# bytedance/particle-sfm

Hardware: AMD Instinct MI355X
Metric: trajectory-points/s (higher is better)
Workload: dtype f32 sampling + f64 positions; 1 GPU; configs[1]: synthetic 100x(1920x1080) flow pairs, sample_ratio=2, flow_check + chaining + occlusion + id assignment, 1 sequence per GPU; frames=101, height=1080, width=1920, trajectories=2073277, parallelism=sequence-per-gpu x1, world_size=1

## Files before the change

### include/psfm.h

```cpp
#ifndef PSFM_H_
#define PSFM_H_

#include <stddef.h>
#include <stdint.h>

#ifdef __cplusplus
extern "C" {
#endif

#define PSFM_VERSION 141

typedef enum psfm_status {
    PSFM_OK = 0,
    PSFM_ERR_ARG = 1,
    PSFM_ERR_HIP = 2,
    PSFM_ERR_CAPACITY = 3,
    PSFM_ERR_SOLVER = 4
} psfm_status;

typedef struct psfm_ctx psfm_ctx;

enum {
    PSFM_TERM_FUNCTION_TOL = 0,
    PSFM_TERM_PARAMETER_TOL = 1,
// ... 45 lines not shown
                                int w, const float* thres, int pair0, int n_pairs, uint8_t* const* kill_out, void* stream);

psfm_status psfm_ctx_set_solver(psfm_ctx* ctx, int mode, int k);
psfm_status psfm_solver_counters(psfm_ctx* ctx, int64_t* fused, int64_t* fused_redone, int64_t* chain, int32_t* k_now);

psfm_status psfm_ctx_set_resident_budget(psfm_ctx* ctx, int blocks);
psfm_status psfm_resident_capacity(psfm_ctx* ctx, int32_t* blocks);

psfm_status psfm_solver_launches(psfm_ctx* ctx, int64_t* resident, int64_t* giveups, int64_t* iterations);

psfm_status psfm_flow_check(psfm_ctx* ctx, const float* flows_f, const float* flows_b, int n_pairs, int h,
                            int w, float thres, uint8_t* occ_out, float* err_out, void* stream);

psfm_status psfm_load_flo_stack(psfm_ctx* ctx, const char* const* paths_host, int n, int h, int w, float* dst, int n_threads, void* stream);

psfm_status psfm_grid_sample(psfm_ctx* ctx, const float* map_hwc, int c, int h, int w, const double* xy,
                             int64_t n, float* out, void* stream);

psfm_status psfm_optimize_location(psfm_ctx* ctx, const double* uv12, const double* ref1, const double* ref2,
                                   const double* scale, const float* flow12, int64_t n, int w, int h,
                                   double* out, psfm_solve_stats* stats_host, void* stream);

psfm_status psfm_path_consistency_eval(psfm_ctx* ctx, const double* uv12, const double* ref1, const double* ref2,
                                       const double* scale, const float* flow12, int64_t n, int w, int h,
                                       double* residuals, double* jacobians, void* stream);

psfm_status psfm_sort_records(psfm_ctx* ctx, uint32_t* keys, int32_t* values, int64_t n, int end_bit, void* stream);

psfm_status psfm_sort_records64(psfm_ctx* ctx, uint64_t* keys, int32_t* values, int64_t n, int end_bit, void* stream);

psfm_status psfm_ctx_get_finalize_forms(psfm_ctx* ctx, int* sort_form, int* offsets_form);

psfm_status psfm_ctx_get_finalize_placed(psfm_ctx* ctx, int* placed);

psfm_status psfm_track(psfm_ctx* ctx, const float* flows, const uint8_t* occ, const float* flows_f2,
                       const uint8_t* occ_s2, int n_flows, int h, int w, int sample_ratio,
                       psfm_track_info* info_host, void* stream);

psfm_status psfm_connect(psfm_ctx* ctx, const float* flows_f, const float* flows_b, const float* flows_f2,
                         const float* flows_b2, int n_flows, int h, int w, float thres, int sample_ratio,
                         uint8_t* occ, uint8_t* occ_s2, psfm_track_info* info_host, void* stream);

psfm_status psfm_track_queries(psfm_ctx* ctx, const float* flows_f, const uint8_t* occ_f, const float* flows_b, const uint8_t* occ_b,
                               int n_flows, int h, int w, const double* q_xy, const int32_t* q_t, int64_t n_q,
                               psfm_track_info* info_host, void* stream);

psfm_status psfm_track_queries_optimize(psfm_ctx* ctx, const float* flows_f, const uint8_t* occ_f, const float* flows_f2,
                                        const uint8_t* occ_f2, const float* flows_b, const uint8_t* occ_b, const float* flows_b2,
                                        const uint8_t* occ_b2, int n_flows, int h, int w, const double* q_xy, const int32_t* q_t,
                                        int64_t n_q, psfm_track_info* info_host, void* stream);

psfm_status psfm_track_queries_batch(psfm_ctx* const* ctxs, int n_seq, const float* const* flows_f, const uint8_t* const* occ_f,
                                     const float* const* flows_b, const uint8_t* const* occ_b, const int* n_flows, const int* h,
                                     const int* w, const double* const* q_xy, const int32_t* const* q_t, const int64_t* n_q,
                                     psfm_track_info* infos_host, void* stream);
psfm_status psfm_query_batch_census(psfm_ctx* ctx, int32_t* launches, int32_t* host_syncs);

psfm_status psfm_track_queries_optimize_batch(psfm_ctx* const* ctxs, int n_seq, const float* const* flows_f, const uint8_t* const* occ_f,
                                              const float* const* flows_f2, const uint8_t* const* occ_f2, const float* const* flows_b,
                                              const uint8_t* const* occ_b, const float* const* flows_b2, const uint8_t* const* occ_b2,
                                              const int* n_flows, const int* h, const int* w, const double* const* q_xy,
                                              const int32_t* const* q_t, const int64_t* n_q, psfm_track_info* infos_host, void* stream);
psfm_status psfm_query_pc_batch_census(psfm_ctx* ctx, int32_t* launches_fixed, int32_t* launches_iter, int32_t* host_syncs);

psfm_status psfm_connect_batch(psfm_ctx* const* ctxs, int n_seq, const float* const* flows_f, const float* const* flows_b,
                               const float* const* flows_f2, const float* const* flows_b2, const int* n_flows, int h, int w,
// ... 151 lines not shown
```

### particle-sfm_amd/csrc/psfm_api.hip

```cpp
#include <stdarg.h>
#include <stdio.h>
#include <string.h>
#include <mutex>
#include <shared_mutex>
#include <atomic>
#include <chrono>
#include <stdlib.h>

#include "psfm_internal.h"
#include "psfm_solve_policy.h"

static thread_local char g_err[512] = "";
static std::shared_mutex g_dev_gate[16];
std::shared_mutex& psfm_device_gate(int device) { return g_dev_gate[device & 15]; }
static std::atomic<int> g_dev_waiters[16];
int psfm_gate_waiters(int device) { return g_dev_waiters[device & 15].load(std::memory_order_relaxed); }
void psfm_gate_waiters_add(int device, int d) { g_dev_waiters[device & 15].fetch_add(d, std::memory_order_relaxed); }
static int psfm_wants_persist(psfm_ctx* c, bool optimize, int h, int w, int ratio, bool fused)
{
    if (c->chain_mode == 1 || ratio < 1 || !psfm_frame_ok(h, w)) return 0;
    if (c->mb_enable && !optimize) return 0;
    if (optimize) return c->resident_budget > 0 ? 0 : 1;
    const int64_t G = (int64_t)((w + ratio - 1) / ratio) * ((h + ratio - 1) / ratio);
    const int64_t P = (int64_t)h * w;
// ... 351 lines not shown
        return PSFM_ERR_ARG;
    }
    if (n == 0) return PSFM_OK;
    hipStream_t s = (hipStream_t)stream;
    psfm_status st;
    if ((st = c->sort_keys.ensure(sizeof(unsigned long long) * (size_t)n * 2)) != PSFM_OK) return st;
    if ((st = c->sort_lanes.ensure(sizeof(int) * (size_t)n * 2)) != PSFM_OK) return st;
    const int64_t half = psfm_sort_pairs64_passes((unsigned)end_bit) % 2 == 0 ? 0 : n;
    unsigned long long* k0 = c->sort_keys.as<unsigned long long>();
    int* v0 = c->sort_lanes.as<int>();
    PSFM_HIP(hipMemcpyAsync(k0 + half, keys, sizeof(unsigned long long) * (size_t)n, hipMemcpyDeviceToDevice, s));
    PSFM_HIP(hipMemcpyAsync(v0 + half, values, sizeof(int) * (size_t)n, hipMemcpyDeviceToDevice, s));
    if ((st = psfm_sort_pairs64(c, k0, v0, k0 + n, v0 + n, n, (unsigned)end_bit, s)) != PSFM_OK) return st;
    PSFM_HIP(hipMemcpyAsync(keys, k0, sizeof(unsigned long long) * (size_t)n, hipMemcpyDeviceToDevice, s));
    PSFM_HIP(hipMemcpyAsync(values, v0, sizeof(int) * (size_t)n, hipMemcpyDeviceToDevice, s));
    return PSFM_OK;
}

extern "C" psfm_status psfm_ctx_get_finalize_forms(psfm_ctx* c, int* sort_form, int* offsets_form)
{
    PSFM_CHECK_CTX(c);
    if (sort_form) *sort_form = c->fin_sort_form;
    if (offsets_form) *offsets_form = c->fin_offsets_form;
    return PSFM_OK;
}

extern "C" psfm_status psfm_ctx_get_finalize_placed(psfm_ctx* c, int* placed)
{
    PSFM_CHECK_CTX(c);
    if (placed) *placed = c->fin_placed;
    return PSFM_OK;
}

psfm_status psfm_track_dims(psfm_ctx* c, int n_flows, int h, int w, int ratio, int64_t g_own, PsfmTrackDims& d)
{
    d.H = h; d.W = w; d.ratio = ratio; d.n_flows = n_flows;
    d.GW = (w + ratio - 1) / ratio; d.GH = (h + ratio - 1) / ratio;
    d.G = (int64_t)d.GW * d.GH;
    const int64_t Gown = g_own < 0 ? d.G : (g_own > 0 ? g_own : 1);
    d.cap = (int64_t)(c->lane_factor * (double)Gown);
    d.cap = ((d.cap + 255) / 256) * 256;
    const int64_t n_blocks = d.cap / 256;
    {
        const int64_t gb = (Gown + 255) / 256;
        d.nsh = (int)(gb < PSFM_NSHARD ? (gb > 0 ? gb : 1) : PSFM_NSHARD);
    }
    d.free_cap = (int)(((n_blocks + d.nsh - 1) / d.nsh) * 256) + 1024;
    const double tf = c->traj_factor > (double)n_flows / 8.0 ? c->traj_factor : (double)n_flows / 8.0;
    d.shard_cap = (int)(((int64_t)(tf * (double)Gown) + d.cap) / d.nsh) + 1024;
    d.traj_cap = (int64_t)d.shard_cap * PSFM_NSHARD;
    if (d.cap > 0x7fffffff / 2 || d.traj_cap > 0x7fffffff / 2) { psfm_set_error("psfm_track: grid too large"); return PSFM_ERR_ARG; }
    d.shift_b = 1; while ((1ll << d.shift_b) < d.G) ++d.shift_b;
    int tbits = 1; while ((1ll << tbits) < (long long)n_flows + 2) ++tbits;
    d.shift_d = d.shift_b + tbits;
    if (d.shift_d + tbits > 63) { psfm_set_error("psfm_track: key does not fit 64 bits"); return PSFM_ERR_ARG; }
    d.cw = (float)((double)(w - 1) / 2.0); d.ch = (float)((double)(h - 1) / 2.0);
    return PSFM_OK;
}

psfm_status psfm_track_alloc(psfm_ctx* c, const PsfmTrackDims& d)
{
    psfm_status st;
    const int n_flows = d.n_flows;
    if ((st = c->log.ensure(sizeof(double2) * (size_t)(n_flows + 1) * d.cap)) != PSFM_OK) return st;
    if ((st = c->birth_frame.ensure(sizeof(int) * d.cap)) != PSFM_OK) return st;
    if ((st = c->birth_idx.ensure(sizeof(int) * d.cap)) != PSFM_OK) return st;
// ... 429 lines not shown
```

### particle-sfm_amd/csrc/psfm_finalize.hip

```cpp
#include <cstring>
#include <stdio.h>
#include <rocprim/device/device_radix_sort.hpp>
#include <rocprim/device/device_scan.hpp>

#include "psfm_device.h"
#include "psfm_finalize_plan.h"
#include "psfm_internal.h"
#include "psfm_place.h"

#define PSFM_BLOCK 256

__device__ __forceinline__ void psfm_collect_alive_body(
    const int* __restrict__ birth_frame, const int* __restrict__ birth_idx, PsfmCounters* __restrict__ ctr,
    PsfmShard* __restrict__ shards, unsigned long long* __restrict__ fin_keys, int* __restrict__ fin_lanes, int cap,
    int shard_cap, int last_time, int shift_b, int shift_d)
{
    __shared__ int s_cnt[PSFM_BLOCK / PSFM_WAVE];
    __shared__ int s_base;
    const int n_lanes = min(ctr->n_lanes, cap);
    if ((int)(blockIdx.x * PSFM_BLOCK) >= n_lanes) return;
    const int i = blockIdx.x * PSFM_BLOCK + threadIdx.x;
    int bf = -1;
    if (i < n_lanes) bf = birth_frame[i];
    const bool pending = bf <= -2;
    const bool alive = (bf >= 0) | pending;
    const int my_last = pending ? last_time - 1 : last_time;
    if (pending) bf = -2 - bf;
    const unsigned long long am = __ballot(alive);
    const int lane = psfm_lane_id(), wave = threadIdx.x / PSFM_WAVE;
    if (lane == 0) s_cnt[wave] = __popcll(am);
    __syncthreads();
    const int shard = blockIdx.x % PSFM_NSHARD;
    if (threadIdx.x == 0) {
        int tot = 0;
        for (int w = 0; w < PSFM_BLOCK / PSFM_WAVE; ++w) tot += s_cnt[w];
        s_base = tot > 0 ? atomicAdd(&shards[shard].fin_cnt, tot) : 0;
    }
    __syncthreads();
    if (alive) {
// ... 280 lines not shown
        r[u] = (t >= 1 && t < lj) ? dlog[(int64_t)(bj + t - 1) * cap + col] : make_float2(0.f, 0.f);
    }
    if (tid < TILE_J) s_off[tid] = id0 + tid < n ? psfm_track_offset(pl, off, id0 + tid, hb, hl) : 0;
    for (int k0 = 0; k0 < maxlen; k0 += TILE_K) {
#pragma unroll
        for (int u = 0; u < NLD; ++u) dtile[j][q + u * (PSFM_BLOCK / TILE_J)] = r[u];
        __syncthreads();
        if (k0 + TILE_K < maxlen) {
#pragma unroll
            for (int u = 0; u < NLD; ++u) {
                const int t = k0 + TILE_K + q + u * (PSFM_BLOCK / TILE_J);
                r[u] = (t < lj) ? dlog[(int64_t)(bj + t - 1) * cap + col] : make_float2(0.f, 0.f);
            }
        }
        if (tid < TILE_J) {
            double2 pos = s_pos[tid];
            const int l = s_len[tid];
            float2 f[TILE_K];
#pragma unroll
            for (int k = 0; k < TILE_K; ++k) f[k] = dtile[tid][k];
#pragma unroll
            for (int k = 0; k < TILE_K; ++k) {
                const int t = k0 + k;
                if (t >= 1 && t < l) { pos.x = pos.x + (double)f[k].x; pos.y = pos.y + (double)f[k].y; }
                tile[tid][k] = pos;
            }
            s_pos[tid] = pos;
        }
        __syncthreads();
        const int kk = tid & (TILE_K - 1);
        for (int jj = tid / TILE_K; jj < TILE_J; jj += PSFM_BLOCK / TILE_K) {
            const int t = k0 + kk;
            if (t < s_len[jj]) out[s_off[jj] + t] = tile[jj][kk];
        }
        __syncthreads();
    }
}

static PsfmFinForm psfm_form_of(const PsfmTrackDims& d, int64_t n, int n_seq = 0)
{
    static const int sort_on = getenv("PSFM_FIN_SORT") ? atoi(getenv("PSFM_FIN_SORT")) : 1;
    static const int plan_on = getenv("PSFM_FIN_PLAN") ? atoi(getenv("PSFM_FIN_PLAN")) : 1;
    return psfm_fin_form(d.shift_b, d.shift_d, d.n_flows, n_seq > 0 ? n_seq : 1, n, sort_on, plan_on, n_seq > 0 ? 0 : 1);
}

struct PsfmFinDst { unsigned long long* keys; int* lanes; };
static PsfmFinDst psfm_compact_dst(psfm_ctx* c, const PsfmFinForm& f, int64_t n)
{
    const int64_t half = f.first_half ? 0 : n;
    return {f.fmt.use32 ? (unsigned long long*)(c->sort_keys.as<unsigned>() + half) : c->sort_keys.as<unsigned long long>() + half,
            c->sort_lanes.as<int>() + half};
}

template <class K>
static psfm_status psfm_rocprim_sort(psfm_ctx* c, int64_t n, unsigned end_bit, size_t scan_bytes, hipStream_t s)
{
    K* k_out = c->sort_keys.as<K>(), *k_in = k_out + n;
    int* l_out = c->sort_lanes.as<int>(), *l_in = l_out + n;
    size_t tmp_bytes = 0;
    psfm_status st;
    PSFM_HIP(rocprim::radix_sort_pairs(nullptr, tmp_bytes, k_in, k_out, l_in, l_out, (size_t)n, 0u, end_bit, s));
    if ((st = c->sort_tmp.ensure(tmp_bytes > scan_bytes ? tmp_bytes : scan_bytes)) != PSFM_OK) return st;
    PSFM_HIP(rocprim::radix_sort_pairs(c->sort_tmp.p, tmp_bytes, k_in, k_out, l_in, l_out, (size_t)n, 0u, end_bit, s));
    return PSFM_OK;
}

// ... 43 lines not shown
    const long long ng = f.ng;
    const PsfmKeyFmt fmt = f.fmt;
    PsfmPlan pl;
    pl.gstart = nullptr; pl.goff = nullptr; pl.keys = (const void*)c->sort_keys.p; pl.use32 = fmt.use32; pl.shift_b = d.shift_b; pl.shift_d = d.shift_d;
    pl.birth_w = c->res_birth.as<int>(); pl.len_w = c->res_len.as<int>(); pl.off_w = c->res_off.as<int64_t>();
    if (f.offsets_form == 1) {
        if ((st = c->scan_tmp.ensure((sizeof(int64_t) + sizeof(int)) * (size_t)ng)) != PSFM_OK) return st;
        int64_t* goff = c->scan_tmp.as<int64_t>();
        int* gstart = (int*)(goff + ng);
        const void* had = c->fin_marks.p;
        if ((st = c->fin_marks.ensure(sizeof(int) * (size_t)PSFM_PLAN_MAX_GROUPS)) != PSFM_OK) return st;
        if (!c->fin_marks_clean || had != c->fin_marks.p)
            PSFM_HIP(hipMemsetAsync(c->fin_marks.p, 0xff, sizeof(int) * (size_t)PSFM_PLAN_MAX_GROUPS, s));
        c->fin_marks_clean = false;
        hipLaunchKernelGGL(psfm_group_bounds_kernel, dim3((unsigned)((n + PSFM_BLOCK - 1) / PSFM_BLOCK)), dim3(PSFM_BLOCK), 0, s,
                           (const void*)c->sort_keys.p, n, fmt.use32, d.shift_b, d.shift_d, c->fin_marks.as<int>());
        hipLaunchKernelGGL(psfm_group_plan_kernel, dim3(1), dim3(PSFM_PLAN_BLOCK), 0, s, c->fin_marks.as<int>(), gstart, goff, (int)ng, n,
                           c->res_off.as<int64_t>() + n);
        PSFM_HIP(hipGetLastError());
        c->fin_marks_clean = true;
        c->fin_offsets_form = 1;
        pl.gstart = gstart; pl.goff = goff;
    } else {
        c->fin_offsets_form = 3;
        if ((st = c->scan_tmp.ensure(sizeof(int64_t) * (n + 1))) != PSFM_OK) return st;
        hipLaunchKernelGGL(psfm_decode_kernel, dim3((unsigned)((n + 1 + PSFM_BLOCK - 1) / PSFM_BLOCK)), dim3(PSFM_BLOCK), 0, s,
                           (const void*)c->sort_keys.p, n, fmt, c->res_birth.as<int>(), c->res_len.as<int>(), c->scan_tmp.as<int64_t>());
        PSFM_HIP(hipGetLastError());
        PSFM_HIP(rocprim::exclusive_scan(c->sort_tmp.p, scan_bytes, c->scan_tmp.as<int64_t>(), c->res_off.as<int64_t>(),
                                         (int64_t)0, (size_t)(n + 1), rocprim::plus<int64_t>(), s));
    }
    c->res_n_points = npts;
    if ((st = c->res_xy.ensure(sizeof(double2) * (size_t)(npts > 0 ? npts : 1))) != PSFM_OK) return st;
    if (delta_log)
        hipLaunchKernelGGL(psfm_gather_delta_kernel, dim3((unsigned)((n + TILE_J - 1) / TILE_J)), dim3(PSFM_BLOCK), 0, s,
                           c->log.as<float2>(), d.cap, c->sort_lanes.as<int>(), c->res_birth.as<int>(),
                           c->res_len.as<int>(), c->res_off.as<int64_t>(), n, (const void*)c->sort_keys.p, fmt.use32,
                           d.shift_b, d.GW, d.ratio, c->res_xy.as<double2>(), pl);
    else
        hipLaunchKernelGGL(psfm_gather_kernel, dim3((unsigned)((n + TILE_J - 1) / TILE_J)), dim3(PSFM_BLOCK), 0, s,
                           c->log.as<double2>(), d.cap, c->sort_lanes.as<int>(), c->res_birth.as<int>(),
                           c->res_len.as<int>(), c->res_off.as<int64_t>(), n, c->res_xy.as<double2>(), pl);
    PSFM_HIP(hipGetLastError());
    return PSFM_OK;
}

psfm_status psfm_finalize(psfm_ctx* c, const PsfmTrackDims& d, hipStream_t s)
{
    PsfmCounters* ctr = c->counters.as<PsfmCounters>();
    PsfmShard* shards = c->shards.as<PsfmShard>();
    hipLaunchKernelGGL(psfm_collect_alive_kernel, dim3((unsigned)((d.cap + PSFM_BLOCK - 1) / PSFM_BLOCK)), dim3(PSFM_BLOCK),
                       0, s, c->birth_frame.as<int>(), c->birth_idx.as<int>(), ctr, shards,
                       c->fin_keys.as<unsigned long long>(), c->fin_lanes.as<int>(), (int)d.cap, d.shard_cap,
                       d.n_flows, d.shift_b, d.shift_d);
    PSFM_HIP(hipGetLastError());
    PsfmCounters* hc = (PsfmCounters*)c->host_pinned;
    PsfmShard* hs = psfm_host_shards(c);
    PSFM_HIP(hipMemcpyAsync(hc, ctr, sizeof(PsfmCounters), hipMemcpyDeviceToHost, s));
    PSFM_HIP(hipMemcpyAsync(hs, shards, sizeof(PsfmShard) * PSFM_NSHARD, hipMemcpyDeviceToHost, s));
    PSFM_HIP(hipStreamSynchronize(s));
    PsfmShardOffsets so;
    int fin_cnt[PSFM_NSHARD];
    int64_t n = 0, npts = 0;
    for (int k = 0; k < PSFM_NSHARD; ++k) { npts += hs[k].points; fin_cnt[k] = hs[k].fin_cnt; }
    const bool over = psfm_shard_offsets(fin_cnt, d.shard_cap, &so, &n) || hc->overflow != 0;
    if (over || hc->n_lanes > d.cap) {
        psfm_set_error("capacity exceeded: lanes used %d of %lld, trajectory records %lld of %lld (%d shards); "
                       "raise psfm_ctx_set_capacity", hc->n_lanes, (long long)d.cap, (long long)n,
                       (long long)d.traj_cap, PSFM_NSHARD);
        return PSFM_ERR_CAPACITY;
    }
    c->res_n_traj = n;
// ... 270 lines not shown
```

### particle-sfm_amd/csrc/psfm_internal.h

```cpp
#pragma once
#include <hip/hip_runtime.h>
#include <stdint.h>
#include <string.h>
#include <shared_mutex>
#include <string>
#include <vector>

#include "../../include/psfm.h"

#define PSFM_MAX_PEERS 8

void psfm_set_error(const char* fmt, ...);

#define PSFM_HIP(expr)                                                                          \
    do {                                                                                        \
        hipError_t e_ = (expr);                                                                 \
        if (e_ != hipSuccess) {                                                                 \
            psfm_set_error("%s failed: %s (%s:%d)", #expr, hipGetErrorString(e_), __FILE__, __LINE__); \
            return PSFM_ERR_HIP;                                                                \
        }                                                                                       \
    } while (0)

static inline bool psfm_frame_ok(int h, int w) { return h >= 2 && w >= 2 && (int64_t)h * (int64_t)w * 8 < ((int64_t)1 << 32); }

// ... 81 lines not shown

struct PsfmTrackDims;

struct psfm_ctx {
    int device = 0;
    double lane_factor = 2.0, traj_factor = 8.0;
    PsfmBuf log;
    PsfmBuf birth_frame;
    PsfmBuf birth_idx;
    PsfmBuf free_stack;
    PsfmBuf fin_keys;
    PsfmBuf fin_lanes;
    PsfmBuf occupied;
    PsfmBuf counters;
    PsfmBuf shards;
    PsfmBuf survivors;
    PsfmBuf handoff;
    PsfmBuf seg_info;
    PsfmBuf seg_table;
    PsfmBuf persist_bar;
    PsfmBuf place_tab;
    int persist_max_blocks = -1;
    int chain_mode = 0;
    bool mb_enable = false;
    float mb_thres = 0.02f;
    PsfmBuf kill;
    void* host_seg = nullptr;
    size_t host_seg_bytes = 0;
    PsfmBuf sort_keys, sort_lanes, sort_tmp, scan_tmp;
    PsfmBuf fin_marks;
    bool fin_marks_clean = false;
    int fin_sort_form = 0, fin_offsets_form = 0;
    int fin_placed = 0;
    PsfmBuf res_birth, res_len, res_off, res_xy;
    int64_t res_n_traj = 0, res_n_points = 0;
    int res_n_flows = 0;
    bool res_is_query = false;
    PsfmBuf qr_ws;
    PsfmBuf qb_tab, qb_ws;
    void* qb_host = nullptr;
    int32_t qb_launches = 0, qb_syncs = 0;
    PsfmBuf qpb_tab, qpb_ws, qpb_owner;
    void* qpb_host = nullptr;
    int32_t qpb_fixed = 0, qpb_iter = 0, qpb_syncs = 0;
    PsfmBuf sol_x, sol_state, sol_partials, sol_ctrl, sol_misc, sol_stats, sol_fused, sol_bar;
    PsfmBuf sol_list;
    int pc_persist_blocks[4] = {-1, -1, -1, -1};
    bool pc_persist_ok = false;
    int resident_budget = 0;
    unsigned pc_epoch = 0;
    PsfmBuf peer_area;
    unsigned peer_epoch = 0;
    int peer_world = 0, peer_rank = 0;
    int peer_L[PSFM_MAX_PEERS] = {0};
    void* peer_lead[PSFM_MAX_PEERS] = {nullptr};
    void* peer_opened[PSFM_MAX_PEERS] = {nullptr};
    int pc_giveups = 0;
    int solve_K = 4;
    int solve_mode = 0;
    int solver_mode = 0, solver_K = 0;
    int64_t n_fused_ok = 0, n_fused_redone = 0, n_chain = 0;
    int64_t n_resident = 0, n_iter_launches = 0;
    PsfmTrackDims* shard_dims = nullptr;
    bool shard_optimize = false;
    int solve_unroll = 6;
    PsfmBuf occ_own, occ2_own;
// ... 286 lines not shown
```

### particle-sfm_amd/point_trajectory/_hip.py

```python
import ctypes
import os

_PKG = os.path.dirname(os.path.dirname(os.path.abspath(__file__)))
LIB_PATH = os.environ.get("PSFM_HIP_LIB", os.path.join(_PKG, "lib", "libpsfm_hip.so"))

PSFM_OK, PSFM_ERR_ARG, PSFM_ERR_HIP, PSFM_ERR_CAPACITY, PSFM_ERR_SOLVER = 0, 1, 2, 3, 4
PROF_KINDS = {"flow_check": 0, "chain_step": 1, "respawn": 2, "solver": 3, "finalize": 4}

EXPORTS = [
    "psfm_last_error", "psfm_version", "psfm_device_count", "psfm_ctx_create", "psfm_ctx_destroy",
    "psfm_ctx_set_capacity", "psfm_flow_check", "psfm_grid_sample", "psfm_optimize_location", "psfm_track",
    "psfm_connect",
    "psfm_result_device", "psfm_result_copy", "psfm_result_solve_stats", "psfm_ctx_set_profiling",
    "psfm_profile_get", "psfm_ctx_set_chain_mode", "psfm_window_sample", "psfm_result_filter", "psfm_result_filtered_copy",
    "psfm_ctx_set_solver", "psfm_solver_counters", "psfm_traj_to_matches", "psfm_matches_copy",
    "psfm_shard_begin", "psfm_shard_step", "psfm_shard_solve_export", "psfm_shard_solve_control", "psfm_shard_solve_restore",
    "psfm_shard_solve_writeback", "psfm_shard_solve_record", "psfm_shard_finish", "psfm_result_keys",
    "psfm_shard_solve_control_async", "psfm_shard_window_state", "psfm_shard_peek_stall", "psfm_shard_frame",
    "psfm_shard_solve_control_chain_async", "psfm_shard_solve_poll", "psfm_shard_solve_local", "psfm_shard_solve_redo_local", "psfm_connect_batch", "psfm_solver_launches", "psfm_ctx_set_resident_budget", "psfm_resident_capacity", "psfm_load_flo_stack",
    "psfm_path_consistency_eval", "psfm_sort_records", "psfm_sort_records64", "psfm_ctx_get_finalize_forms", "psfm_ctx_get_finalize_placed",
    "psfm_shard_peer_area", "psfm_shard_peer_epoch", "psfm_shard_peer_open", "psfm_shard_peer_connect", "psfm_shard_solve_blocks", "psfm_shard_solve_peer",
    "psfm_labels_begin", "psfm_labels_merge_window", "psfm_labels_finish", "psfm_labels_device", "psfm_labels_copy", "psfm_labels_to_matches",
    "psfm_traj_augment", "psfm_traj_encode_weight_count", "psfm_traj_encode",
    "psfm_traj_decode_weight_count", "psfm_traj_decode_workspace_bytes", "psfm_traj_decode",
    "psfm_traj_decode_batch_workspace_bytes", "psfm_traj_decode_batch",
    "psfm_window_sample_batch", "psfm_traj_augment_batch", "psfm_traj_encode_batch",
    "psfm_traj_eval_counts", "psfm_traj_vote_labels",
    "psfm_labels_set", "psfm_matches_to_database", "psfm_database_copy", "psfm_database_chunk_rows",
    "psfm_database_compact_again",
    "psfm_sparse_depth", "psfm_sparse_depth_sort_ids", "psfm_ctx_set_sparse_depth", "psfm_ctx_get_sparse_depth_budget",
    "psfm_sparse_depth_last_ms", "psfm_colmap_points3d_count", "psfm_colmap_points3d_scan",
    "psfm_ctx_set_motion_boundary", "psfm_motion_boundary", "psfm_kill_map", "psfm_kill_map_batch",
    "psfm_depth_display", "psfm_ctx_set_depth_display", "psfm_depth_display_last_ms", "psfm_depth_display_chunk",
    "psfm_track_queries", "psfm_track_queries_optimize",
    "psfm_result_filter_batch", "psfm_traj_to_matches_batch", "psfm_labels_to_matches_batch", "psfm_matches_batch_census", "psfm_labels_sizes",
    "psfm_track_queries_batch", "psfm_query_batch_census",
    "psfm_track_queries_optimize_batch", "psfm_query_pc_batch_census",
    "psfm_ctx_set_batch_redo", "psfm_connect_batch_census", "psfm_ctx_set_frame_size",
]


class SolveStats(ctypes.Structure):
    _fields_ = [("iterations", ctypes.c_int32), ("successful_steps", ctypes.c_int32),
                ("termination", ctypes.c_int32), ("dogleg_nonGN", ctypes.c_int32),
                ("initial_cost", ctypes.c_double), ("final_cost", ctypes.c_double)]

    def as_dict(self):
        return {k: getattr(self, k) for k, _ in self._fields_}


class TrackInfo(ctypes.Structure):
    _fields_ = [("n_traj", ctypes.c_int64), ("n_points", ctypes.c_int64), ("n_lanes_peak", ctypes.c_int64),
                ("lane_capacity", ctypes.c_int64), ("solver_iterations", ctypes.c_int64),
                ("n_solves", ctypes.c_int32), ("chain_mode", ctypes.c_int32)]

    def as_dict(self):
        return {k: getattr(self, k) for k, _ in self._fields_}


class PsfmError(RuntimeError):
    def __init__(self, status, msg):
        super().__init__("libpsfm_hip status %d: %s" % (status, msg))
        self.status = status


_lib = None


def lib():
    global _lib
    if _lib is not None:
        return _lib
    if not os.path.exists(LIB_PATH):
        raise RuntimeError(
            "libpsfm_hip.so not found at %s -- build it with `python particle-sfm_amd/build.py` "
            "(the HIP extension is mandatory, there is no CPU fallback)" % LIB_PATH)
    import torch
    L = ctypes.CDLL(LIB_PATH)
    vp, i32, i64, f32, f64 = ctypes.c_void_p, ctypes.c_int, ctypes.c_int64, ctypes.c_float, ctypes.c_double
    L.psfm_last_error.restype = ctypes.c_char_p
    L.psfm_last_error.argtypes = []
    L.psfm_version.restype = i32
    L.psfm_device_count.restype = i32
    L.psfm_ctx_create.argtypes = [i32, ctypes.POINTER(vp)]
    L.psfm_ctx_destroy.argtypes = [vp]
    L.psfm_ctx_set_capacity.argtypes = [vp, f64, f64]
    L.psfm_load_flo_stack.argtypes = [vp, ctypes.POINTER(ctypes.c_char_p), i32, i32, i32, vp, i32, vp]
    L.psfm_flow_check.argtypes = [vp, vp, vp, i32, i32, i32, f32, vp, vp, vp]
    L.psfm_grid_sample.argtypes = [vp, vp, i32, i32, i32, vp, i64, vp, vp]
    L.psfm_optimize_location.argtypes = [vp, vp, vp, vp, vp, vp, i64, i32, i32, vp, ctypes.POINTER(SolveStats), vp]
    L.psfm_path_consistency_eval.argtypes = [vp, vp, vp, vp, vp, vp, i64, i32, i32, vp, vp, vp]
    L.psfm_sort_records.argtypes = [vp, vp, vp, i64, i32, vp]
    L.psfm_sort_records64.argtypes = [vp, vp, vp, i64, i32, vp]
    L.psfm_ctx_get_finalize_forms.argtypes = [vp, ctypes.POINTER(ctypes.c_int32), ctypes.POINTER(ctypes.c_int32)]
    L.psfm_ctx_get_finalize_placed.argtypes = [vp, ctypes.POINTER(ctypes.c_int32)]
    L.psfm_track.argtypes = [vp, vp, vp, vp, vp, i32, i32, i32, i32, ctypes.POINTER(TrackInfo), vp]
    L.psfm_connect.argtypes = [vp, vp, vp, vp, vp, i32, i32, i32, f32, i32, vp, vp, ctypes.POINTER(TrackInfo), vp]
    L.psfm_connect_batch.argtypes = [ctypes.POINTER(vp), i32, ctypes.POINTER(vp), ctypes.POINTER(vp), ctypes.POINTER(vp), ctypes.POINTER(vp),
                                     ctypes.POINTER(i32), i32, i32, f32, i32, ctypes.POINTER(TrackInfo), vp]
    L.psfm_ctx_set_batch_redo.argtypes = [vp, i32]
    L.psfm_ctx_set_frame_size.argtypes = [vp, i32, i32]
    L.psfm_connect_batch_census.argtypes = [vp] + [ctypes.POINTER(ctypes.c_int32)] * 5
    L.psfm_track_queries.argtypes = [vp, vp, vp, vp, vp, i32, i32, i32, vp, vp, i64, ctypes.POINTER(TrackInfo), vp]
    L.psfm_track_queries_optimize.argtypes = [vp, vp, vp, vp, vp, vp, vp, vp, vp, i32, i32, i32, vp, vp, i64, ctypes.POINTER(TrackInfo), vp]
    L.psfm_track_queries_batch.argtypes = [ctypes.POINTER(vp), i32, ctypes.POINTER(vp), ctypes.POINTER(vp), ctypes.POINTER(vp), ctypes.POINTER(vp),
                                           ctypes.POINTER(i32), ctypes.POINTER(i32), ctypes.POINTER(i32), ctypes.POINTER(vp), ctypes.POINTER(vp),
                                           ctypes.POINTER(i64), ctypes.POINTER(TrackInfo), vp]
    L.psfm_query_batch_census.argtypes = [vp, ctypes.POINTER(ctypes.c_int32), ctypes.POINTER(ctypes.c_int32)]
    L.psfm_track_queries_optimize_batch.argtypes = [ctypes.POINTER(vp), i32] + [ctypes.POINTER(vp)] * 8 + [
        ctypes.POINTER(i32), ctypes.POINTER(i32), ctypes.POINTER(i32), ctypes.POINTER(vp), ctypes.POINTER(vp), ctypes.POINTER(i64),
        ctypes.POINTER(TrackInfo), vp]
    L.psfm_query_pc_batch_census.argtypes = [vp, ctypes.POINTER(ctypes.c_int32), ctypes.POINTER(ctypes.c_int32), ctypes.POINTER(ctypes.c_int32)]
    L.psfm_result_device.argtypes = [vp, ctypes.POINTER(vp), ctypes.POINTER(vp), ctypes.POINTER(vp), ctypes.POINTER(vp)]
    L.psfm_result_copy.argtypes = [vp, vp, vp, vp, vp, vp]
    L.psfm_result_solve_stats.argtypes = [vp, ctypes.POINTER(SolveStats), i32, ctypes.POINTER(ctypes.c_int32)]
    L.psfm_ctx_set_profiling.argtypes = [vp, i32]
    L.psfm_ctx_set_chain_mode.argtypes = [vp, i32]
    L.psfm_ctx_set_solver.argtypes = [vp, i32, i32]
    L.psfm_ctx_set_motion_boundary.argtypes = [vp, i32, f32]
    L.psfm_motion_boundary.argtypes = [vp, vp, i32, i32, i32, f32, vp, vp]
    L.psfm_kill_map.argtypes = [vp, vp, vp, i32, i32, i32, f32, vp, vp]
    L.psfm_kill_map_batch.argtypes = [vp, ctypes.POINTER(vp), ctypes.POINTER(vp), ctypes.POINTER(i32), i32, i32, i32, ctypes.POINTER(f32), i32, i32,
                                      ctypes.POINTER(vp), vp]
    L.psfm_solver_counters.argtypes = [vp, ctypes.POINTER(i64), ctypes.POINTER(i64), ctypes.POINTER(i64), ctypes.POINTER(ctypes.c_int32)]
    L.psfm_ctx_set_resident_budget.argtypes = [vp, i32]
    L.psfm_resident_capacity.argtypes = [vp, ctypes.POINTER(ctypes.c_int32)]
    L.psfm_solver_launches.argtypes = [vp, ctypes.POINTER(i64), ctypes.POINTER(i64), ctypes.POINTER(i64)]
    L.psfm_result_filter.argtypes = [vp, i32, ctypes.POINTER(i64), ctypes.POINTER(i64), vp]
# ... 124 lines not shown
    def connect_batch_census(self):
        v = [ctypes.c_int32() for _ in range(5)]
        check(lib().psfm_connect_batch_census(self._h, *[ctypes.byref(x) for x in v]))
        return dict(zip(("n_left", "n_together", "launches_fixed", "launches_iter", "host_syncs"), (int(x.value) for x in v)))

    def set_resident_budget(self, blocks):
        check(lib().psfm_ctx_set_resident_budget(self._h, int(blocks)))
        self.resident_budget = int(blocks)

    def resident_capacity(self):
        n = ctypes.c_int32()
        check(lib().psfm_resident_capacity(self._h, ctypes.byref(n)))
        return int(n.value)

    def solver_counters(self):
        a, b, c_, k = ctypes.c_int64(), ctypes.c_int64(), ctypes.c_int64(), ctypes.c_int32()
        check(lib().psfm_solver_counters(self._h, ctypes.byref(a), ctypes.byref(b), ctypes.byref(c_), ctypes.byref(k)))
        out = {"fused": a.value, "fused_redone": b.value, "chain": c_.value, "k": k.value}
        r, g, it = ctypes.c_int64(), ctypes.c_int64(), ctypes.c_int64()
        check(lib().psfm_solver_launches(self._h, ctypes.byref(r), ctypes.byref(g), ctypes.byref(it)))
        out.update({"resident_launches": r.value, "resident_giveups": g.value, "iteration_launches": it.value})
        return out

    def finalize_forms(self):
        a, b = ctypes.c_int32(), ctypes.c_int32()
        check(lib().psfm_ctx_get_finalize_forms(self._h, ctypes.byref(a), ctypes.byref(b)))
        return {"sort": int(a.value), "offsets": int(b.value)}

    def finalize_placed(self):
        a = ctypes.c_int32()
        check(lib().psfm_ctx_get_finalize_placed(self._h, ctypes.byref(a)))
        return int(a.value)

    def query_batch_census(self):
        a, b = ctypes.c_int32(), ctypes.c_int32()
        check(lib().psfm_query_batch_census(self._h, ctypes.byref(a), ctypes.byref(b)))
        return {"launches": int(a.value), "host_syncs": int(b.value)}

    def query_pc_batch_census(self):
        a, b, c = ctypes.c_int32(), ctypes.c_int32(), ctypes.c_int32()
        check(lib().psfm_query_pc_batch_census(self._h, ctypes.byref(a), ctypes.byref(b), ctypes.byref(c)))
        return {"launches_fixed": int(a.value), "launches_iter": int(b.value), "host_syncs": int(c.value)}

    def set_sparse_depth(self, budget_bytes=1 << 30, timing=False):
        check(lib().psfm_ctx_set_sparse_depth(self._h, int(budget_bytes), int(bool(timing))))

    def sparse_depth_ms(self):
        ms = (ctypes.c_double * 3)()
        check(lib().psfm_sparse_depth_last_ms(self._h, ms))
        return {"fill_ms": ms[0], "winner_ms": ms[1], "store_ms": ms[2]}

    def set_depth_display(self, timing=False):
        check(lib().psfm_ctx_set_depth_display(self._h, int(bool(timing))))

    def depth_display_ms(self):
        ms = (ctypes.c_double * 4)()
        check(lib().psfm_depth_display_last_ms(self._h, ms))
        return {"count_ms": ms[0], "compact_ms": ms[1], "select_ms": ms[2], "colour_ms": ms[3]}

    def set_profiling(self, enable):
        check(lib().psfm_ctx_set_profiling(self._h, int(enable)))

    def profile(self):
        out = {}
        for name, k in PROF_KINDS.items():
            ms, n = ctypes.c_double(), ctypes.c_int64()
# ... 74 lines not shown
```

Before: 22.69 billion trajectory-points/s.

## Parallelize finalize delta-gather prefix sum with DPP wave scan and exactness fallback

```diff
diff --git a/include/psfm.h b/include/psfm.h
--- a/include/psfm.h
+++ b/include/psfm.h
@@ -101,6 +101,8 @@
 psfm_status psfm_ctx_get_finalize_forms(psfm_ctx* ctx, int* sort_form, int* offsets_form);
 
 psfm_status psfm_ctx_get_finalize_placed(psfm_ctx* ctx, int* placed);
+
+psfm_status psfm_ctx_get_finalize_gather(psfm_ctx* ctx, int* gather);
 
 psfm_status psfm_track(psfm_ctx* ctx, const float* flows, const uint8_t* occ, const float* flows_f2,
                        const uint8_t* occ_s2, int n_flows, int h, int w, int sample_ratio,
diff --git a/particle-sfm_amd/csrc/psfm_api.hip b/particle-sfm_amd/csrc/psfm_api.hip
--- a/particle-sfm_amd/csrc/psfm_api.hip
+++ b/particle-sfm_amd/csrc/psfm_api.hip
@@ -407,6 +407,13 @@
     return PSFM_OK;
 }
 
+extern "C" psfm_status psfm_ctx_get_finalize_gather(psfm_ctx* c, int* gather)
+{
+    PSFM_CHECK_CTX(c);
+    if (gather) *gather = c->fin_gather;
+    return PSFM_OK;
+}
+
 psfm_status psfm_track_dims(psfm_ctx* c, int n_flows, int h, int w, int ratio, int64_t g_own, PsfmTrackDims& d)
 {
     d.H = h; d.W = w; d.ratio = ratio; d.n_flows = n_flows;
diff --git a/particle-sfm_amd/csrc/psfm_finalize.hip b/particle-sfm_amd/csrc/psfm_finalize.hip
--- a/particle-sfm_amd/csrc/psfm_finalize.hip
+++ b/particle-sfm_amd/csrc/psfm_finalize.hip
@@ -5,6 +5,7 @@
 
 #include "psfm_device.h"
 #include "psfm_finalize_plan.h"
+#include "psfm_gather_exact.h"
 #include "psfm_internal.h"
 #include "psfm_place.h"
 
@@ -351,6 +352,137 @@
         for (int jj = tid / TILE_K; jj < TILE_J; jj += PSFM_BLOCK / TILE_K) {
             const int t = k0 + kk;
             if (t < s_len[jj]) out[s_off[jj] + t] = tile[jj][kk];
+        }
+        __syncthreads();
+    }
+}
+
+
+template <int D>
+__device__ __forceinline__ double psfm_gx_row_shr(double v)
+{
+    const long long b = __double_as_longlong(v);
+    const int lo = __builtin_amdgcn_update_dpp(0, (int)(unsigned)(b & 0xffffffffll), 0x110 + D, 0xf, 0xf, false);
+    const int hi = __builtin_amdgcn_update_dpp(0, (int)(b >> 32), 0x110 + D, 0xf, 0xf, false);
+    return __longlong_as_double(((long long)hi << 32) | (long long)(unsigned)lo);
+}
+__device__ __forceinline__ double psfm_gx_row_bcast15(double v)
+{
+    const long long b = __double_as_longlong(v);
+    const int lo = __builtin_amdgcn_update_dpp(0, (int)(unsigned)(b & 0xffffffffll), 0x142, 0xa, 0xf, false);
+    const int hi = __builtin_amdgcn_update_dpp(0, (int)(b >> 32), 0x142, 0xa, 0xf, false);
+    return __longlong_as_double(((long long)hi << 32) | (long long)(unsigned)lo);
+}
+__device__ __forceinline__ double psfm_gx_scan32(double v)
+{
+    v = v + psfm_gx_row_shr<1>(v);
+    v = v + psfm_gx_row_shr<2>(v);
+    v = v + psfm_gx_row_shr<4>(v);
+    v = v + psfm_gx_row_shr<8>(v);
+    return v + psfm_gx_row_bcast15(v);
+}
+
+#ifdef PSFM_GX_COUNT
+__device__ unsigned long long psfm_gx_counts[2];
+extern "C" int psfm_gx_read_counts(unsigned long long* out)
+{
+    return hipMemcpyFromSymbol(out, HIP_SYMBOL(psfm_gx_counts), sizeof(unsigned long long) * 2) == hipSuccess ? 0 : 1;
+}
+#endif
+
+__global__ __launch_bounds__(PSFM_BLOCK) void psfm_gather_delta2_kernel(const float2* __restrict__ dlog, int64_t cap,
+                                                                        const int* __restrict__ lanes,
+                                                                        const int* __restrict__ birth,
+                                                                        const int* __restrict__ len,
+                                                                        const int64_t* __restrict__ off, int64_t n,
+                                                                        const void* __restrict__ keys, int use32, int shift_b,
+                                                                        int GW, int ratio, double2* __restrict__ out, PsfmPlan pl)
+{
+    static_assert(TILE_K == PSFM_GX_CHUNK && PSFM_WAVE == 2 * TILE_K, "a half-wave sums one trajectory's chunk");
+    __shared__ float2 dtile[TILE_J][TILE_K + 1];
+    __shared__ double2 s_pos[TILE_J];
+    __shared__ int s_lane[TILE_J], s_birth[TILE_J], s_len[TILE_J], s_sticky[TILE_J];
+    __shared__ int64_t s_off[TILE_J];
+    __shared__ int s_maxlen;
+    const int tid = threadIdx.x;
+    const int64_t id0 = (int64_t)blockIdx.x * TILE_J;
+    int hb = 0, hl = 0;
+    if (tid == 0) s_maxlen = 0;
+    __syncthreads();
+    if (tid < TILE_J) {
+        const int64_t id = id0 + tid;
+        const bool ok = id < n;
+        int b = 0, l = 0, idx = -1;
+        const int my_lane = ok ? lanes[id] : 0;
+        if (ok) psfm_track_header(pl, birth, len, id, &b, &l, &idx);
+        hb = b; hl = l;
+        s_lane[tid] = my_lane;
+        s_birth[tid] = b;
+        s_len[tid] = l;
+        s_sticky[tid] = 0;
+        double2 p0 = make_double2(0.0, 0.0);
+        if (ok) {
+            atomicMax(&s_maxlen, l);
+            if (idx < 0) idx = psfm_key_idx(psfm_key_at(keys, id, use32), shift_b);
+            const int gy = idx / GW, gx = idx - gy * GW;
+            p0 = make_double2((double)(gx * ratio), (double)(gy * ratio));
+        }
+        s_pos[tid] = p0;
+    }
+    __syncthreads();
+    const int maxlen = s_maxlen;
+    const int j = tid & (TILE_J - 1);
+    const int q = tid / TILE_J;
+    constexpr int NLD = TILE_K * TILE_J / PSFM_BLOCK;
+    const int lj = s_len[j];
+    const int64_t col = s_lane[j];
+    const int bj = s_birth[j];
+    float2 r[NLD];
+#pragma unroll
+    for (int u = 0; u < NLD; ++u) {
+        const int t = q + u * (PSFM_BLOCK / TILE_J);
+        r[u] = (t >= 1 && t < lj) ? dlog[(int64_t)(bj + t - 1) * cap + col] : make_float2(0.f, 0.f);
+    }
+    if (tid < TILE_J) s_off[tid] = id0 + tid < n ? psfm_track_offset(pl, off, id0 + tid, hb, hl) : 0;
+    const int kk = tid & (TILE_K - 1);
+    const int half = tid & TILE_K;
+    for (int k0 = 0; k0 < maxlen; k0 += TILE_K) {
+#pragma unroll
+        for (int u = 0; u < NLD; ++u) dtile[j][q + u * (PSFM_BLOCK / TILE_J)] = r[u];
+        __syncthreads();
+        if (k0 + TILE_K < maxlen) {
+#pragma unroll
+            for (int u = 0; u < NLD; ++u) {
+                const int t = k0 + TILE_K + q + u * (PSFM_BLOCK / TILE_J);
+                r[u] = (t < lj) ? dlog[(int64_t)(bj + t - 1) * cap + col] : make_float2(0.f, 0.f);
+            }
+        }
+        const int t = k0 + kk;
+        for (int jj = tid / TILE_K; jj < TILE_J; jj += PSFM_BLOCK / TILE_K) {
+            const int l = s_len[jj];
+            if (__builtin_amdgcn_ballot_w64(k0 < l) == 0ull) continue;
+            float2 f = dtile[jj][kk];
+            if (!(t >= 1 && t < l)) f = make_float2(0.f, 0.f);
+            const double2 base = s_pos[jj];
+            const int sticky = s_sticky[jj];
+            double2 p = make_double2(base.x + psfm_gx_scan32((double)f.x), base.y + psfm_gx_scan32((double)f.y));
+            const unsigned fine = (unsigned)(__builtin_amdgcn_ballot_w64(psfm_gx_class2(f) != 0) >> half);
+            const unsigned inr = (unsigned)(__builtin_amdgcn_ballot_w64(psfm_gx_in_range(p.x, p.y) != 0) >> half);
+            const int par = psfm_gx_chunk_parallel(sticky, fine == 0xffffffffu, inr == 0xffffffffu);
+#ifdef PSFM_GX_COUNT
+            if (kk == 0 && k0 < l) { atomicAdd(&psfm_gx_counts[0], 1ull); if (!par) atomicAdd(&psfm_gx_counts[1], 1ull); }
+#endif
+            if (__builtin_amdgcn_ballot_w64(!par) != 0ull) {
+                double2 run = base, mine = base;
+                for (int s = 0; s < TILE_K; ++s) {
+                    const float fx = __shfl(f.x, s, TILE_K), fy = __shfl(f.y, s, TILE_K);
+                    run.x = run.x + (double)fx; run.y = run.y + (double)fy;
+                    if (s == kk) mine = run;
+                }
+                if (!par) p = mine;
+            }
+            if (t < l) out[s_off[jj] + t] = p;
+            if (kk == TILE_K - 1) { s_pos[jj] = p; s_sticky[jj] = par ? 0 : 1; }
         }
         __syncthreads();
     }
@@ -460,12 +592,16 @@
     }
     c->res_n_points = npts;
     if ((st = c->res_xy.ensure(sizeof(double2) * (size_t)(npts > 0 ? npts : 1))) != PSFM_OK) return st;
-    if (delta_log)
-        hipLaunchKernelGGL(psfm_gather_delta_kernel, dim3((unsigned)((n + TILE_J - 1) / TILE_J)), dim3(PSFM_BLOCK), 0, s,
-                           c->log.as<float2>(), d.cap, c->sort_lanes.as<int>(), c->res_birth.as<int>(),
+    c->fin_gather = 0;
+    if (delta_log) {
+        static const int gather_on = getenv("PSFM_FIN_GATHER") ? atoi(getenv("PSFM_FIN_GATHER")) : 1;
+        const int gx = psfm_gx_form(gather_on, d.H, d.W);
+        hipLaunchKernelGGL(gx ? psfm_gather_delta2_kernel : psfm_gather_delta_kernel, dim3((unsigned)((n + TILE_J - 1) / TILE_J)),
+                           dim3(PSFM_BLOCK), 0, s, c->log.as<float2>(), d.cap, c->sort_lanes.as<int>(), c->res_birth.as<int>(),
                            c->res_len.as<int>(), c->res_off.as<int64_t>(), n, (const void*)c->sort_keys.p, fmt.use32,
                            d.shift_b, d.GW, d.ratio, c->res_xy.as<double2>(), pl);
-    else
+        c->fin_gather = gx ? 2 : 1;
+    } else
         hipLaunchKernelGGL(psfm_gather_kernel, dim3((unsigned)((n + TILE_J - 1) / TILE_J)), dim3(PSFM_BLOCK), 0, s,
                            c->log.as<double2>(), d.cap, c->sort_lanes.as<int>(), c->res_birth.as<int>(),
                            c->res_len.as<int>(), c->res_off.as<int64_t>(), n, c->res_xy.as<double2>(), pl);
diff --git a/particle-sfm_amd/csrc/psfm_gather_exact.h b/particle-sfm_amd/csrc/psfm_gather_exact.h
--- /dev/null
+++ b/particle-sfm_amd/csrc/psfm_gather_exact.h
@@ -0,0 +1,35 @@
+#pragma once
+#include <hip/hip_runtime.h>
+#include <stdint.h>
+#include <string.h>
+
+#ifndef PSFM_HD
+#define PSFM_HD __host__ __device__ __forceinline__
+#endif
+
+#define PSFM_GX_CHUNK 32
+#define PSFM_GX_EXP_LO (127 - 17)
+#define PSFM_GX_EXP_HI (127 + 8)
+#define PSFM_GX_POS_LIMIT 8192.0
+#define PSFM_GX_MAX_FRAME ((1 << 12) - (1 << 8))
+
+PSFM_HD int psfm_gx_class(float f)
+{
+    unsigned u;
+    memcpy(&u, &f, sizeof(u));
+    const unsigned e = (u >> 23) & 0xffu;
+    return ((u << 1) == 0u || (e >= (unsigned)PSFM_GX_EXP_LO && e < (unsigned)PSFM_GX_EXP_HI)) ? 1 : 0;
+}
+PSFM_HD int psfm_gx_class2(float2 f) { return psfm_gx_class(f.x) & psfm_gx_class(f.y); }
+
+PSFM_HD int psfm_gx_in_range(double x, double y)
+{
+    return (x > -PSFM_GX_POS_LIMIT && x < PSFM_GX_POS_LIMIT && y > -PSFM_GX_POS_LIMIT && y < PSFM_GX_POS_LIMIT) ? 1 : 0;
+}
+
+PSFM_HD int psfm_gx_chunk_parallel(int sticky, int all_fine, int all_in_range) { return (!sticky && all_fine && all_in_range) ? 1 : 0; }
+
+static inline int psfm_gx_form(int gather_switch, int H, int W)
+{
+    return (gather_switch && H <= PSFM_GX_MAX_FRAME && W <= PSFM_GX_MAX_FRAME) ? 1 : 0;
+}
diff --git a/particle-sfm_amd/csrc/psfm_internal.h b/particle-sfm_amd/csrc/psfm_internal.h
--- a/particle-sfm_amd/csrc/psfm_internal.h
+++ b/particle-sfm_amd/csrc/psfm_internal.h
@@ -137,6 +137,7 @@
     bool fin_marks_clean = false;
     int fin_sort_form = 0, fin_offsets_form = 0;
     int fin_placed = 0;
+    int fin_gather = 0;
     PsfmBuf res_birth, res_len, res_off, res_xy;
     int64_t res_n_traj = 0, res_n_points = 0;
     int res_n_flows = 0;
diff --git a/particle-sfm_amd/point_trajectory/_hip.py b/particle-sfm_amd/point_trajectory/_hip.py
--- a/particle-sfm_amd/point_trajectory/_hip.py
+++ b/particle-sfm_amd/point_trajectory/_hip.py
@@ -37,6 +37,7 @@
     "psfm_track_queries_batch", "psfm_query_batch_census",
     "psfm_track_queries_optimize_batch", "psfm_query_pc_batch_census",
     "psfm_ctx_set_batch_redo", "psfm_connect_batch_census", "psfm_ctx_set_frame_size",
+    "psfm_ctx_get_finalize_gather",
 ]
 
 
@@ -94,6 +95,7 @@
     L.psfm_sort_records64.argtypes = [vp, vp, vp, i64, i32, vp]
     L.psfm_ctx_get_finalize_forms.argtypes = [vp, ctypes.POINTER(ctypes.c_int32), ctypes.POINTER(ctypes.c_int32)]
     L.psfm_ctx_get_finalize_placed.argtypes = [vp, ctypes.POINTER(ctypes.c_int32)]
+    L.psfm_ctx_get_finalize_gather.argtypes = [vp, ctypes.POINTER(ctypes.c_int32)]
     L.psfm_track.argtypes = [vp, vp, vp, vp, vp, i32, i32, i32, i32, ctypes.POINTER(TrackInfo), vp]
     L.psfm_connect.argtypes = [vp, vp, vp, vp, vp, i32, i32, i32, f32, i32, vp, vp, ctypes.POINTER(TrackInfo), vp]
     L.psfm_connect_batch.argtypes = [ctypes.POINTER(vp), i32, ctypes.POINTER(vp), ctypes.POINTER(vp), ctypes.POINTER(vp), ctypes.POINTER(vp),
@@ -284,6 +286,11 @@
         check(lib().psfm_ctx_get_finalize_placed(self._h, ctypes.byref(a)))
         return int(a.value)
 
+    def finalize_gather(self):
+        a = ctypes.c_int32()
+        check(lib().psfm_ctx_get_finalize_gather(self._h, ctypes.byref(a)))
+        return int(a.value)
+
     def query_batch_census(self):
         a, b = ctypes.c_int32(), ctypes.c_int32()
         check(lib().psfm_query_batch_census(self._h, ctypes.byref(a), ctypes.byref(b)))
```

After: 23.06 billion trajectory-points/s, median of 6. +1.6%, better.
